# mct10/Speech-Vecalign

Hardware: AMD Instinct MI355X
Metric: aligned doc-pairs/sec (higher is better)
Workload: dtype bf16; 1 GPU; synthetic 4096x4096 d=1024 bf16 embeddings, 4 overlap layers/side, 10 alignment types, band 14, coarse-to-fine (max_size_full_dp=300), 1024 doc-pairs per GPU per step; pipeline=1, N=4096, M=4096, d=1024, overlaps=4, parallelism=dp1 (pairs sharded, no collective)

## Files before the change

### speech-vecalign_amd/csrc/svx_api.hip

```cpp
#include <stdarg.h>
#include <stdio.h>
#include <stdlib.h>
#include <string.h>

#include <chrono>
#include <functional>
#include <memory>
#include <type_traits>
#include <vector>

#include "svx_common.h"

static char g_err[512] = "";

int svx_fail(svx_ctx* ctx, int code, const char* fmt, ...) {
    char* dst = ctx ? ctx->err : g_err;
    va_list ap;
    va_start(ap, fmt);
    vsnprintf(dst, 512, fmt, ap);
    va_end(ap);
    return code;
}

static const char* kStageNames[] = {"pyr0",       "pyrN",     "pyr_aux",      "knob_scoresN", "knob",      "dense_costs",
// ... 796 lines not shown
static int next_event(svx_ctx* ctx, hipEvent_t* out) {
    svx_ctx_ext* cx = X(ctx);
    if (cx->ev_pool.size() < 256) {
        hipEvent_t e;
        SVX_HIP(ctx, hipEventCreateWithFlags(&e, hipEventDisableTiming));
        cx->ev_pool.push_back(e);
        *out = e;
        return SVX_OK;
    }
    *out = cx->ev_pool[cx->ev_next++ % cx->ev_pool.size()];
    return SVX_OK;
}

static void front_ops(svx_ctx* ctx, HalfState& H, std::vector<Op>& ops, int split) {
    svx_ctx_ext* cx = X(ctx);
    HalfState* h = &H;
    const BatchParams& bp = H.bp;
    const int np = H.n_pairs, d = bp.d, dtype = bp.dtype;
    const double waves = (double)((np + 1023) / 1024);
    const int parts = (split > 1 && np >= 16 * split) ? split : 1;
    struct Evs { hipEvent_t pass[SVX_MAX_LEVELS][8]; };
    auto evs = std::make_shared<Evs>();
    ops.push_back({0.0, -1, [=]() -> int {
        SVX_HIP(ctx, hipEventRecord(cx->side_fork, ctx->stream));
        SVX_HIP(ctx, hipStreamWaitEvent(cx->side, cx->side_fork, 0));
        SVX_HIP(ctx, hipStreamWaitEvent(cx->helper, cx->side_fork, 0));
        return SVX_OK;
    }});
    auto sort_op = [=]() -> int {
        hipStream_t main_stream = ctx->stream;
        static const bool inline_sort = getenv("SVX_SORT_INLINE") != nullptr;
        if (parts > 1 && !inline_sort) SVX_HIP(ctx, hipStreamWaitEvent(cx->side, evs->pass[0][parts - 1], 0));
        ctx->stream = inline_sort ? main_stream : cx->side;
        int rc;
        {
            StageScope sc(ctx, S_KNOB_SORT);
            rc = svxl_knob_scores(ctx, h->dpairs, np, h->maxL, h->max_kn, h->max_n0, dtype, d, 0);
        }
        ctx->stream = main_stream;
        if (rc) return rc;
        SVX_HIP(ctx, hipEventRecord(cx->side_join, inline_sort ? main_stream : cx->side));
        return SVX_OK;
    };
    if (parts == 1) ops.push_back({0.0, -1, sort_op});
    for (int l = 0; l <= H.maxL; l++) {
        for (int q = 0; q < parts; q++) {
            const int lo = (int)((long long)np * q / parts), hi = (int)((long long)np * (q + 1) / parts);
            const double aux_us = (l == 0 ? 700.0 * waves : 250.0) / parts;
            if (parts == 1) {
                ops.push_back({aux_us, S_PYR_AUX, [=]() { return svxl_pyramid_level(ctx, h->dpairs, np, l, dtype, d, h->max_nblk[l], h->max_ksum, 0); }});
                ops.push_back({H.b_pyr[l] / (l == 0 ? 4.9e6 : 5.3e6), l == 0 ? S_PYR0 : (l == 1 ? S_PYR1 : S_PYRN),
                               [=]() { return svxl_pyramid_level(ctx, h->dpairs, np, l, dtype, d, h->max_nblk[l], h->max_ksum, 1); }});
                continue;
            }
            ops.push_back({H.b_pyr[l] / (l == 0 ? 4.9e6 : 5.3e6) / parts, l == 0 ? S_PYR0 : (l == 1 ? S_PYR1 : S_PYRN), [=]() -> int {
                hipStream_t main_stream = ctx->stream;
                int rc;
                if (l == 0 && q == 0) {
                    StageScope sc(ctx, S_PYR_AUX);
                    if ((rc = svxl_pyramid_level(ctx, h->dpairs + lo, hi - lo, l, dtype, d, h->max_nblk[l], h->max_ksum, 0))) return rc;
                } else {
                    if (l > 0) SVX_HIP(ctx, hipStreamWaitEvent(cx->helper, evs->pass[l - 1][q], 0));
                    ctx->stream = cx->helper;
                    {
                        StageScope sc(ctx, S_PYR_AUX);
                        rc = svxl_pyramid_level(ctx, h->dpairs + lo, hi - lo, l, dtype, d, h->max_nblk[l], h->max_ksum, 0);
                    }
                    ctx->stream = main_stream;
                    if (rc) return rc;
                    hipEvent_t aux_done;
                    if ((rc = next_event(ctx, &aux_done))) return rc;
                    SVX_HIP(ctx, hipEventRecord(aux_done, cx->helper));
                    SVX_HIP(ctx, hipStreamWaitEvent(main_stream, aux_done, 0));
                }
                if ((rc = svxl_pyramid_level(ctx, h->dpairs + lo, hi - lo, l, dtype, d, h->max_nblk[l], h->max_ksum, 1))) return rc;
                if ((rc = next_event(ctx, &evs->pass[l][q]))) return rc;
                SVX_HIP(ctx, hipEventRecord(evs->pass[l][q], main_stream));
                return SVX_OK;
            }});
        }
        if (parts > 1 && l == 0) ops.push_back({0.0, -1, sort_op});
    }
    if (!bp.straight) {
        ops.push_back({H.dense_cells * 2.7e-5, S_DENSE_COSTS, [=]() -> int {
            int rc = svxl_dense_costs_batch(ctx, h->dpairs, np, h->max_ds0, h->max_ds1, dtype, d);
            if (rc) return rc;
            return svxl_knob_from_dots(ctx, h->dpairs, np, h->max_kn);
        }});
    }
    if (H.maxL >= 1) {
        ops.push_back({H.b_knobN / 16.5e6, S_KNOB_SCORES, [=]() -> int {
            SVX_HIP(ctx, hipStreamWaitEvent(ctx->stream, cx->side_join, 0));
            return svxl_knob_scores(ctx, h->dpairs, np, h->maxL, h->max_kn, h->max_n0, dtype, d, 1);
        }});
    }
    ops.push_back({H.b_knob0 / 8.5e6, S_KNOB_SCORES0, [=]() -> int {
        SVX_HIP(ctx, hipStreamWaitEvent(ctx->stream, cx->side_join, 0));
        return svxl_knob_scores(ctx, h->dpairs, np, h->maxL, h->max_kn, h->max_n0, dtype, d, 2);
    }});
}

struct Seg {
    std::vector<Op> lb;
    bool has_s = false;
    Op s;
};

static void chain_segs(svx_ctx* ctx, HalfState& H, std::vector<Seg>& segs) {
    HalfState* h = &H;
    const BatchParams bp = H.bp;
    const int np = H.n_pairs, d = bp.d, dtype = bp.dtype, W = bp.W, B = bp.B;
    const double waves = (double)((np + 1023) / 1024);
    Seg cur;
    cur.lb.push_back({(np * (H.maxL + 1) * 0.21 < 300.0 ? 300.0 : np * (H.maxL + 1) * 0.21), S_KNOB,
                      [=]() { return svxl_del_penalty_batch(ctx, h->dpairs, np, h->maxL + 1, bp.frac); }});
    if (!bp.straight)
        cur.lb.push_back({(H.max_ds0 + H.max_ds1) * 1.7 * waves, S_DENSE_DP, [=]() { return svxl_dense_stage_batch(ctx, h->dpairs, np, h->max_ds0); }});
    const int first_depth = H.maxL > 0 ? H.maxL - 1 : 0;
    for (int depth = first_depth; depth >= 0; depth--) {
        const SvxTypes ty = depth == 0 ? bp.tfinal : bp.t11;
        int lim2 = 0, tamax2 = 0;
        const bool v2 = !bp.tiles && svxl_band2_limits(ty, W, depth, dtype, d, &lim2, &tamax2);
        const int maxA = H.max_A[depth];
        const int src_rows = (H.maxL > 0 && !H.any_L0) ? maxA / 2 + 8 : maxA;
        cur.lb.push_back({maxA * 0.08 * waves + 60.0, depth == 0 ? S_PATH0 : S_PATH, [=]() {
            return svxl_search_path_batch(ctx, h->dpairs, np, depth, maxA, src_rows, v2 ? lim2 : SVX_BC_ROWS - SVX_BC_TB,
                                          bp.tiles ? 0 : (v2 ? tamax2 : SVX_BC_TAMAX));
        }});
        cur.has_s = true;
        if (bp.tiles) {
            cur.s = {1.0e4, S_TILES, [=]() {
                int* tk = reinterpret_cast<int*>(h->arena + h->o_tickets);
                float* planes = h->b_planes ? reinterpret_cast<float*>(h->arena + h->o_planes) : nullptr;
                return svxl_band_tiles_batch(ctx, h->dpairs, np, ty, W, dtype, h->max_tnd, tk, tk + (size_t)h->max_tnd * np + 1, planes);
            }};
        } else {
            cur.s = {H.b_bc[depth] / 4.0e6, depth == 0 ? S_BAND_COSTS0 : S_BAND_COSTSN, [=]() {
                return v2 ? svxl_band_costs2_batch(ctx, h->dpairs, np, depth, maxA, ty, W, dtype, d)
                          : svxl_band_costs_batch(ctx, h->dpairs, np, depth, maxA, ty, W, dtype, d);
            }};
        }
        segs.push_back(cur);
        cur = Seg();
        if (!bp.tiles)
            cur.lb.push_back({maxA * (0.21 + 0.054 * (ty.n > 1 ? ty.n : 0)) * waves, depth == 0 ? S_BAND_DP0 : S_BAND_DPN,
                              [=]() { return svxl_sparse_dp_batch(ctx, h->dpairs, np, depth, ty, B); }});
        cur.lb.push_back({maxA * 0.27 * waves, depth == 0 ? S_TRACEBACK0 : S_TRACEBACK, [=]() { return svxl_sparse_traceback_batch(ctx, h->dpairs, np, depth, B, maxA, bp.packable ? 1 : 0); }});
    }
    segs.push_back(cur);
}

static int ensure_streams(svx_ctx* ctx) {
    svx_ctx_ext* cx = X(ctx);
    if (!cx->side_ready) {
        int prio_lo = 0, prio_hi = 0;
        SVX_HIP(ctx, hipDeviceGetStreamPriorityRange(&prio_lo, &prio_hi));
        SVX_HIP(ctx, hipStreamCreateWithPriority(&cx->side, hipStreamNonBlocking, prio_lo));
        SVX_HIP(ctx, hipStreamCreateWithPriority(&cx->helper, hipStreamNonBlocking, prio_hi));
        SVX_HIP(ctx, hipEventCreateWithFlags(&cx->side_fork, hipEventDisableTiming));
        SVX_HIP(ctx, hipEventCreateWithFlags(&cx->side_join, hipEventDisableTiming));
        cx->side_ready = true;
    }
    if (!cx->chain_ready) {
        int prio_lo = 0, prio_hi = 0;
        SVX_HIP(ctx, hipDeviceGetStreamPriorityRange(&prio_lo, &prio_hi));
        SVX_HIP(ctx, hipStreamCreateWithPriority(&cx->chain, hipStreamNonBlocking, prio_hi));
        cx->chain_ready = true;
    }
    for (int h = 0; h < 2; h++) {
        if (!cx->half[h].front_done) SVX_HIP(ctx, hipEventCreateWithFlags(&cx->half[h].front_done, hipEventDisableTiming));
        if (!cx->half[h].chain_done) SVX_HIP(ctx, hipEventCreateWithFlags(&cx->half[h].chain_done, hipEventDisableTiming));
        if (!cx->half[h].upload_done) SVX_HIP(ctx, hipEventCreateWithFlags(&cx->half[h].upload_done, hipEventDisableTiming));
    }
    return SVX_OK;
}

static int run_interleaved(svx_ctx* ctx, HalfState* front, HalfState* chain, bool beside) {
    svx_ctx_ext* cx = X(ctx);
    hipStream_t A = ctx->stream, Bst = beside ? cx->chain : ctx->stream;
    std::vector<Op> fops;
    std::vector<Seg> segs;
    if (front) {
        if (front->chain_done_valid) SVX_HIP(ctx, hipStreamWaitEvent(A, front->chain_done, 0));
        {
            StageScope sc(ctx, S_SETUP);
            if (front->upload_valid) SVX_HIP(ctx, hipEventSynchronize(front->upload_done));
            memcpy(front->pinned, front->host.data(), (size_t)front->n_pairs * sizeof(SvxPairDev));
            SVX_HIP(ctx, hipMemcpyAsync(front->dpairs, front->pinned, (size_t)front->n_pairs * sizeof(SvxPairDev), hipMemcpyHostToDevice, A));
            SVX_HIP(ctx, hipEventRecord(front->upload_done, A));
            front->upload_valid = true;
            hipLaunchKernelGGL(k_init_batch, dim3(front->n_pairs), dim3(64), 0, A, front->dpairs);
            SVX_LAUNCH_CHECK(ctx, "k_init_batch");
            if (front->bp.around) {
                int rc = svxl_prior_ingest_batch(ctx, front->dpairs, front->n_pairs);
                if (rc) return rc;
            }
            if (front->bp.nsamp == 0) {
                for (int p = 0; p < front->n_pairs; p++)
                    for (int l = 0; l <= front->host[p].L; l++)
                        for (int s = 0; s < 2; s++)
                            SVX_HIP(ctx, hipMemsetAsync(front->host[p].lev[l].rbar[s], 0, (size_t)front->bp.d * sizeof(float), A));
            }
        }
        static const int split_env = [] { const char* e = getenv("SVX_PIPE_SPLIT"); const int v = e ? atoi(e) : 2; return v >= 1 && v <= 8 ? v : 2; }();
        front_ops(ctx, *front, fops, beside ? split_env : 1);
    }
    if (chain) chain_segs(ctx, *chain, segs);
    int rc;
    size_t fi = 0;
    if (chain && beside) SVX_HIP(ctx, hipStreamWaitEvent(Bst, chain->front_done, 0));
    for (size_t g = 0; g < segs.size(); g++) {
        double need = 0.0;
        for (const Op& op : segs[g].lb) {
            if ((rc = run_op(ctx, op, Bst))) return rc;
            need += op.us;
        }
        hipEvent_t lb_done = nullptr;
        if (beside) {
            if ((rc = next_event(ctx, &lb_done))) return rc;
            SVX_HIP(ctx, hipEventRecord(lb_done, Bst));
// ... 162 lines not shown
```

### speech-vecalign_amd/csrc/svx_band.hip

```cpp
#include <stdlib.h>
#include <string.h>

#include "svx_common.h"

namespace {

typedef __attribute__((ext_vector_type(8))) __bf16 bf16x8_t;
typedef __attribute__((ext_vector_type(8))) _Float16 f16x8_t;
typedef __attribute__((ext_vector_type(4))) float f32x4_t;
typedef __attribute__((address_space(1))) const void* gptr_t;
typedef __attribute__((address_space(3))) void* lptr_t;

constexpr int B2_THREADS = 256;
constexpr int B2_WAVES = 4;
constexpr int B2_TB = 16;
constexpr int B2_SLAB = 64;
constexpr int B2_MAXPASS = 8;
constexpr int B2_MAXSLOT = 20;
constexpr int B2_MAXTPP = 16;

__device__ const uint4 band_zero16[4] = {{0u, 0u, 0u, 0u}, {0u, 0u, 0u, 0u}, {0u, 0u, 0u, 0u}, {0u, 0u, 0u, 0u}};

struct BandPass {
    int t0, nt, nslot;
// ... 222 lines not shown
        auto step = [&](int k, const char* rd, char* wr) {
            if (k < NK) {
                const int younger = (NK - 1 - k) < (S - 2) ? (NK - 1 - k) : (S - 2);
                if (younger >= 2) wait_vm<2 * PW>();
                else if (younger == 1) wait_vm<PW>();
                else wait_vm<0>();
                __builtin_amdgcn_s_barrier();
                asm volatile("" ::: "memory");
                if (k + S - 1 < NK) issue(k + S - 1, wr);
                mma(rd);
            }
        };
        for (int k0 = 0; k0 < NK; k0 += S) {
            if (S == 2) {
                step(k0, st0, st1);
                step(k0 + 1, st1, st0);
            } else if (S == 3) {
                step(k0, st0, st2);
                step(k0 + 1, st1, st0);
                step(k0 + 2, st2, st1);
            } else {
                step(k0, st0, st3);
                step(k0 + 1, st1, st0);
                step(k0 + 2, st2, st1);
                step(k0 + 3, st3, st2);
            }
        }
#pragma unroll
        for (int i = 0; i < SPT; i++) {
            const int r = tid + i * B2_THREADS;
            if (r < NSLOT * ROWS) {
                snrm[r] = r_nrm[i];
                sinv[r] = r_inv[i];
            }
        }
        __syncthreads();
        const float inf = __builtin_inff();
#pragma unroll
        for (int s = 0; s < UPW; s++) {
            const int u = wave + B2_WAVES * s;
            if (u >= nunits) continue;
            const int tl = u / XT, xt = u % XT;
            const int p = ltx[ps.t0 + tl], q = lty[ps.t0 + tl];
            const int xs = (ps.type_slots[tl] & 255) * ROWS, ys = (ps.type_slots[tl] >> 8) * ROWS;
#pragma unroll
            for (int j = 0; j < XT; j++) {
                if (!((umask[s] >> j) & 1)) continue;
                const int yloc = 16 * j + lrow, yy = Y0 + yloc;
                const float ny = snrm[ys + yloc], iy = sinv[ys + yloc];
#pragma unroll
                for (int r = 0; r < 4; r++) {
                    const int xloc = 16 * xt + 4 * lkg + r, xx = X0 + xloc;
                    const int ai = xx + yy - a0;
                    if (ai < 0 || ai >= TAe) continue;
                    const int bi = yy - (spy[ai] - g.W) - b0;
                    if (bi < 0 || bi >= TBe) continue;
                    float c = inf;
                    if (xx >= 0 && xx < g.n && yy >= 0 && yy < g.m) {
                        const float sumx = acc[s][j][r] * sinv[xs + xloc] * iy;
                        c = cost_formula2(sumx, p, q, snrm[xs + xloc], ny);
                    }
                    Fs[(ai * ntp + tl) * TBe + bi] = c;
                }
            }
        }
        __syncthreads();
        if (TBe == B && ntp == g.T && ((g.T * B) & 3) == 0) {
            const int nv = TAe * ntp * TBe / 4;
            float4* dst = reinterpret_cast<float4*>(g.costs + (size_t)a0 * g.T * B);
            const float4* srcv = reinterpret_cast<const float4*>(Fs);
            for (int i = tid; i < nv; i += B2_THREADS) dst[i] = srcv[i];
        } else {
            const int nout = TAe * ntp * TBe;
            for (int idx = tid; idx < nout; idx += B2_THREADS) {
                const int ai = idx / (ntp * TBe);
                const int rem = idx - ai * (ntp * TBe);
                const int tl = rem / TBe, bi = rem - tl * TBe;
                g.costs[((size_t)(a0 + ai) * g.T + ps.t0 + tl) * B + (b0 + bi)] = Fs[idx];
            }
        }
    }
}

template <typename E, bool LV0, int ROWS, int NSLOT, int UPW, int S>
__global__ __launch_bounds__(B2_THREADS) void k_band_costs2(const SvxPairDev* __restrict__ pairs, int depth, SvxTypes ty, BandPlan plan,
                                                            int W, int nchunk_b, int per_pair) {
    using C = Band2<E, ROWS, NSLOT, UPW, S>;
    __shared__ __attribute__((aligned(1024))) char st0[C::STAGE];
    __shared__ __attribute__((aligned(1024))) char st1[C::STAGE];
    __shared__ __attribute__((aligned(1024))) char st2[S >= 3 ? C::STAGE : 16];
    __shared__ __attribute__((aligned(1024))) char st3[S >= 4 ? C::STAGE : 16];
    __shared__ __attribute__((aligned(16))) float Fs[C::FS_FLOATS];
    __shared__ int spx[C::TAMAX + 1], spy[C::TAMAX + 1];
    __shared__ float snrm[NSLOT * ROWS], sinv[NSLOT * ROWS];
    __shared__ int ltx[SVX_MAX_TYPES + 2], lty[SVX_MAX_TYPES + 2];
    __shared__ int tmask[C::XT];
    __shared__ int lslot[NSLOT];
    const unsigned wg = xcd_remap2(blockIdx.x, gridDim.x);
    const SvxPairDev& P = pairs[wg / per_pair];
    const int item = wg % per_pair;
    if (depth > P.L || (depth == P.L && P.L > 0)) return;
    const SvxLevel& Lv = P.lev[depth];
    Band2Args g;
    g.A = *Lv.path_len;
    const int chunk_a = item / nchunk_b;
    if (g.A <= 0 || chunk_a >= *Lv.nchunks) return;
    const int a0 = Lv.cstart[chunk_a], TAe = Lv.cstart[chunk_a + 1] - a0;
    if (TAe <= 0 || TAe > C::TAMAX) return;
    g.n = Lv.n[0];
    g.m = Lv.n[1];
    g.d = P.d;
    g.v0 = LV0 ? P.v[0] : (const void*)Lv.P[0];
    g.v1 = LV0 ? P.v[1] : (const void*)Lv.P[1];
    g.inv0 = LV0 ? Lv.inv[0] : nullptr;
    g.inv1 = LV0 ? Lv.inv[1] : nullptr;
    g.nrm0 = Lv.nrm[0];
    g.nrm1 = Lv.nrm[1];
    g.path = Lv.path;
    g.W = W;
    g.T = ty.n;
    g.costs = Lv.costs;
    g.boff = Lv.boff;
    g.status = P.status;
    band2_block<E, ROWS, NSLOT, UPW, S>(g, ty, plan, a0, TAe, item % nchunk_b, st0, st1, st2, st3, Fs, spx, spy, snrm, sinv, ltx, lty, tmask, lslot);
}

constexpr int B3_THREADS = 512, B3_ROWS = 32, B3_S = 8, B3_G = 2, B3_KX = 4, B3_KY = 4, B3_TMAX = 10;
constexpr int B3_STAGE = B3_KY * B3_ROWS * B2_SLAB;
constexpr int B3_FS = (2 * (B3_ROWS - B2_TB) + 1) * B2_TB * B3_TMAX;

struct BandPlan3 {
    int kx, ky;
    int wt_n[B3_KX];
    int wt_type[B3_KX][B3_KY];
    int wt_yl[B3_KX][B3_KY];
};

template <typename E, int NK, bool AASM, int G>
__device__ void band3_block(const Band2Args& g, const BandPlan3& plan, int a0, int TAe, int chunk_b, char* ring, float* Fs, int* spx,
                            int* spy, float* snrm, float* sinv) {
    using St = typename E::storage;
    static_assert(sizeof(St) == 2, "16-bit rows");
    constexpr int ROWS = B3_ROWS, S = B3_S;
    const int tid = threadIdx.x, lane = tid & 63;
    const int wave = __builtin_amdgcn_readfirstlane(tid >> 6);
    const int xl = wave >> 1, xt = wave & 1;
    const int B = 2 * g.W, b0 = chunk_b * B2_TB;
    const int TBe = (B - b0) < B2_TB ? (B - b0) : B2_TB;
    constexpr int rowbytes = NK * B2_SLAB;
    const int kx = plan.kx, ky = plan.ky;

    if (tid < TAe) {
        const int2 p = reinterpret_cast<const int2*>(g.path)[a0 + tid];
        spx[tid] = p.x;
        spy[tid] = p.y;
    }
    __syncthreads();
    if (tid < TAe) {
        bool ok = (spx[tid] + spy[tid] == a0 + tid);
        if (tid > 0) ok = ok && spx[tid] >= spx[tid - 1] && spy[tid] >= spy[tid - 1];
        if (!ok && g.status) *g.status = SVX_ERR_PATH;
        if (chunk_b == 0) g.boff[a0 + tid] = spy[tid] - g.W;
    }
    const int xlo = spx[0], ylo = spy[0];
    const int X0 = xlo + g.W - (b0 + TBe - 1);
    const int Y0 = ylo - g.W + b0;
    int NXn = spx[TAe - 1] - xlo + TBe, NYn = spy[TAe - 1] - ylo + TBe;
    NXn = NXn < 1 ? 1 : (NXn > ROWS ? ROWS : NXn);
    NYn = NYn < 1 ? 1 : (NYn > ROWS ? ROWS : NYn);

    float r_nrm = 0.f, r_inv = 1.f;
    if (tid < 2 * B3_KX * ROWS) {
        const int side = tid >= B3_KX * ROWS, rr = tid - side * B3_KX * ROWS;
        const int layer = rr / ROWS, loc = rr % ROWS;
        const int gi = (side ? Y0 : X0) + loc, nn = side ? g.m : g.n;
// ... 187 lines not shown
    float* Fs = reinterpret_cast<float*>(ring);
    __shared__ int spx[2 * B3_ROWS], spy[2 * B3_ROWS];
    __shared__ float snrm[2 * B3_KX * B3_ROWS], sinv[2 * B3_KX * B3_ROWS];
    const unsigned wg = xcd_remap2(blockIdx.x, gridDim.x);
    const SvxPairDev& P = pairs[wg / per_pair];
    const int item = wg % per_pair;
    const SvxLevel& Lv = P.lev[0];
    Band2Args g;
    g.A = *Lv.path_len;
    const int chunk_a = item / nchunk_b;
    if (g.A <= 0 || chunk_a >= *Lv.nchunks) return;
    const int a0 = Lv.cstart[chunk_a], TAe = Lv.cstart[chunk_a + 1] - a0;
    if (TAe <= 0 || TAe > 2 * (B3_ROWS - 1) + 1) return;
    g.n = Lv.n[0];
    g.m = Lv.n[1];
    g.d = P.d;
    g.v0 = P.v[0];
    g.v1 = P.v[1];
    g.inv0 = Lv.inv[0];
    g.inv1 = Lv.inv[1];
    g.nrm0 = Lv.nrm[0];
    g.nrm1 = Lv.nrm[1];
    g.path = Lv.path;
    g.W = W;
    g.T = T;
    g.costs = Lv.costs;
    g.boff = Lv.boff;
    g.status = P.status;
    band3_block<E, NK, AASM, G>(g, plan, a0, TAe, item % nchunk_b, ring, Fs, spx, spy, snrm, sinv);
}

bool make_plan3(const SvxTypes& ty, BandPlan3* plan) {
    memset(plan, 0, sizeof(*plan));
    if (ty.n < 1 || ty.n > B3_TMAX) return false;
    for (int t = 0; t < ty.n; t++) {
        const int lx = ty.x[t] - 1, ly = ty.y[t] - 1;
        if (lx >= B3_KX || ly >= B3_KY) return false;
        if (plan->wt_n[lx] >= B3_KY) return false;
        plan->wt_type[lx][plan->wt_n[lx]] = t;
        plan->wt_yl[lx][plan->wt_n[lx]] = ly;
        plan->wt_n[lx]++;
        if (lx + 1 > plan->kx) plan->kx = lx + 1;
        if (ly + 1 > plan->ky) plan->ky = ly + 1;
    }
    return true;
}

int band_version() {
    const char* env = getenv("SVX_BAND_V");
    return env ? atoi(env) : 3;
}

bool make_plan(const SvxTypes& ty, int tpp, int nslot_max, BandPlan* plan) {
    plan->npass = 0;
    int t = 0;
    while (t < ty.n) {
        if (plan->npass >= B2_MAXPASS) return false;
        BandPass& ps = plan->pass[plan->npass];
        memset(&ps, 0, sizeof(ps));
        ps.t0 = t;
        int xs[SVX_MAX_TYPES + 2], ys[SVX_MAX_TYPES + 2];
        memset(xs, 0, sizeof(xs));
        memset(ys, 0, sizeof(ys));
        while (t < ty.n && ps.nt < tpp) {
            const int lx = ty.x[t] - 1, ly = ty.y[t] - 1;
            const int need = (xs[lx] ? 0 : 1) + (ys[ly] ? 0 : 1);
            if (ps.nslot + need > nslot_max) break;
            if (!xs[lx]) { ps.slot_info[ps.nslot] = lx; xs[lx] = ++ps.nslot; }
            if (!ys[ly]) { ps.slot_info[ps.nslot] = (1 << 8) | ly; ys[ly] = ++ps.nslot; }
            ps.type_slots[ps.nt] = (xs[lx] - 1) | ((ys[ly] - 1) << 8);
            ps.nt++;
            t++;
        }
        if (ps.nt == 0) return false;
        plan->npass++;
    }
    return true;
}

struct Variant {
    int rows, nslot, upw, s;
};

bool choose_variant(const SvxTypes& ty, int depth, Variant* v, BandPlan* plan) {
    if (ty.n <= 0) return false;
    int kx = 0, ky = 0;
    for (int t = 0; t < ty.n; t++) {
        if (ty.x[t] > kx) kx = ty.x[t];
        if (ty.y[t] > ky) ky = ty.y[t];
    }
    (void)depth;
    const Variant opts[4] = {{64, 2, 1, 4}, {32, 8, 5, 3}, {32, 12, 8, 3}, {32, 20, 8, 2}};
    for (int i = 0; i < 4; i++) {
        const int tpp = B2_WAVES * opts[i].upw / (opts[i].rows / 16);
        const bool last = i == 3;
        if (!last && (kx + ky > opts[i].nslot || ty.n > tpp)) continue;
        if (!make_plan(ty, tpp, opts[i].nslot, plan)) continue;
        *v = opts[i];
        return true;
    }
    return false;
}

}

static bool use_v3(const SvxTypes& types, int depth, int dtype, int d, BandPlan3* plan3) {
    const int nk3 = d / 32;
    return depth == 0 && dtype != SVX_F32 && band_version() >= 3 && d % 32 == 0 && (nk3 == 32 || nk3 == 16 || nk3 == 8) &&
           make_plan3(types, plan3);
}

bool svxl_band2_limits(const SvxTypes& types, int W, int depth, int dtype, int d, int* lim, int* tamax) {
    const char* env = getenv("SVX_BAND_V1");
    if ((env && atoi(env) != 0) || band_version() <= 1) return false;
    const char* deep = getenv("SVX_BAND_DEEP_V1");
    if (depth > 0 && deep && atoi(deep) != 0) return false;
    Variant v;
    BandPlan plan;
    BandPlan3 plan3;
    if (use_v3(types, depth, dtype, d, &plan3)) v.rows = B3_ROWS;
    else if (!choose_variant(types, depth, &v, &plan)) return false;
    const int B = 2 * W, tbe = B < B2_TB ? B : B2_TB;
    *lim = v.rows - tbe;
    *tamax = 2 * (v.rows - tbe) + 1;
    return true;
}

int svxl_band_costs2_batch(svx_ctx* ctx, const SvxPairDev* pairs, int n_pairs, int depth, int max_A, const SvxTypes& types, int W,
                           int dtype, int d) {
    if (n_pairs <= 0 || max_A <= 0) return SVX_OK;
    BandPlan3 plan3;
    const int nk3 = d / 32;
    if (use_v3(types, depth, dtype, d, &plan3)) {
        const int B3 = 2 * W, tbe3 = B3 < B2_TB ? B3 : B2_TB, lim3 = B3_ROWS - tbe3;
        const int nca3 = (max_A + lim3) / (lim3 + 1), ncb3 = (B3 + B2_TB - 1) / B2_TB;
        dim3 grid3((unsigned)(nca3 * ncb3) * (unsigned)n_pairs);
        const char* aenv = getenv("SVX_BAND_ASMLOAD");
        const bool aasm = aenv ? atoi(aenv) != 0 : true;
#define CALL3(E, NKT)                                                                                                             \
    do {                                                                                                                          \
        if (aasm) hipLaunchKernelGGL((k_band_costs3<E, NKT, true, B3_G>), grid3, dim3(B3_THREADS), 0, ctx->stream, pairs, plan3, types.n, W, ncb3, nca3 * ncb3); \
        else hipLaunchKernelGGL((k_band_costs3<E, NKT, false, B3_G>), grid3, dim3(B3_THREADS), 0, ctx->stream, pairs, plan3, types.n, W, ncb3, nca3 * ncb3); \
    } while (0)
#define CALL3_E(E)                      \
    do {                                \
        if (nk3 == 32) CALL3(E, 32);    \
        else if (nk3 == 16) CALL3(E, 16); \
        else CALL3(E, 8);               \
    } while (0)
        if (dtype == SVX_F16) CALL3_E(ElemF16);
        else CALL3_E(ElemBF16);
#undef CALL3_E
#undef CALL3
        SVX_LAUNCH_CHECK(ctx, "k_band_costs3");
        return SVX_OK;
    }
    Variant v;
    BandPlan plan;
    if (!choose_variant(types, depth, &v, &plan)) return svx_fail(ctx, SVX_ERR_ARG, "band costs: no kernel shape for %d alignment types", types.n);
    const int B = 2 * W, tbe = B < B2_TB ? B : B2_TB;
    const int lim = v.rows - tbe;
    const int nca = (max_A + lim) / (lim + 1), ncb = (B + B2_TB - 1) / B2_TB;
    const int per_pair = nca * ncb;
    dim3 grid((unsigned)per_pair * (unsigned)n_pairs);
    hipStream_t st = ctx->stream;
#define CALL2(E, LV0, ROWS, NSLOT, UPW, S) \
    hipLaunchKernelGGL((k_band_costs2<E, LV0, ROWS, NSLOT, UPW, S>), grid, dim3(B2_THREADS), 0, st, pairs, depth, types, plan, W, ncb, per_pair)
#define CALL2_V(E, LV0)                                      \
    do {                                                     \
        if (v.nslot == 2) CALL2(E, LV0, 64, 2, 1, 4);        \
        else if (v.nslot == 8) CALL2(E, LV0, 32, 8, 5, 3);   \
        else if (v.nslot == 12) CALL2(E, LV0, 32, 12, 8, 3); \
        else CALL2(E, LV0, 32, 20, 8, 2);                    \
    } while (0)
    if (depth > 0) CALL2_V(ElemF32, false);
    else if (dtype == SVX_F32) CALL2_V(ElemF32, true);
    else if (dtype == SVX_F16) CALL2_V(ElemF16, true);
    else CALL2_V(ElemBF16, true);
#undef CALL2_V
#undef CALL2
    SVX_LAUNCH_CHECK(ctx, "k_band_costs2");
    return SVX_OK;
}
```

### speech-vecalign_amd/csrc/svx_costs.hip

```cpp
#include <stdlib.h>

#include "svx_common.h"

namespace {

typedef __attribute__((ext_vector_type(8))) __bf16 bf16x8_t;
typedef __attribute__((ext_vector_type(8))) _Float16 f16x8_t;
typedef __attribute__((ext_vector_type(4))) float f32x4_t;

constexpr int RS = 144;

template <typename E>
struct Mma;
template <>
struct Mma<ElemBF16> {
    static constexpr int KS = 64, NK = 2, KSTEP_BYTES = 64;
    using frag = uint4;
    __device__ static __forceinline__ int lane_off(int lane) { return (lane & 15) * RS + 16 * (lane >> 4); }
    __device__ static __forceinline__ frag load(const char* p) { return *reinterpret_cast<const uint4*>(p); }
    __device__ static __forceinline__ void mma(f32x4_t& acc, const frag& a, const frag& b) {
        acc = __builtin_amdgcn_mfma_f32_16x16x32_bf16(__builtin_bit_cast(bf16x8_t, a), __builtin_bit_cast(bf16x8_t, b), acc, 0, 0, 0);
    }
};
template <>
// ... 57 lines not shown
    const int tid = threadIdx.x, lane = tid & 63, wave = tid >> 6;
    const char** rowptr = reinterpret_cast<const char**>(smem);
    char* slab = smem + 2 * DT * sizeof(char*);
    const int x0 = bx * DT, y0 = by * DT;
    if (tid < 2 * DT) {
        const int side = tid >= DT, loc = tid - side * DT;
        const int gi = (side ? y0 : x0) + loc;
        const int nn = side ? g.s1 : g.s0;
        const char* base = reinterpret_cast<const char*>(side ? g.v1 : g.v0);
        rowptr[tid] = (gi < nn) ? base + (size_t)gi * g.d * sizeof(S) : nullptr;
    }
    f32x4_t acc[2][2];
#pragma unroll
    for (int i = 0; i < 2; i++)
#pragma unroll
        for (int j = 0; j < 2; j++) acc[i][j] = (f32x4_t){0.f, 0.f, 0.f, 0.f};
    const int xt = wave >> 1, yt = wave & 1;
    for (int k0 = 0; k0 < g.d; k0 += Mma<E>::KS) {
        __syncthreads();
        stage_slab<E>(slab, rowptr, 2 * DT, k0, g.d, tid, blockDim.x);
        __syncthreads();
        const char* ap = slab + xt * 32 * RS + Mma<E>::lane_off(lane);
        const char* bp = slab + (DT + yt * 32) * RS + Mma<E>::lane_off(lane);
#pragma unroll
        for (int ks = 0; ks < Mma<E>::NK; ks++) {
            const typename Mma<E>::frag a0 = Mma<E>::load(ap + ks * Mma<E>::KSTEP_BYTES);
            const typename Mma<E>::frag a1 = Mma<E>::load(ap + 16 * RS + ks * Mma<E>::KSTEP_BYTES);
            const typename Mma<E>::frag b0 = Mma<E>::load(bp + ks * Mma<E>::KSTEP_BYTES);
            const typename Mma<E>::frag b1 = Mma<E>::load(bp + 16 * RS + ks * Mma<E>::KSTEP_BYTES);
            Mma<E>::mma(acc[0][0], a0, b0);
            Mma<E>::mma(acc[0][1], a0, b1);
            Mma<E>::mma(acc[1][0], a1, b0);
            Mma<E>::mma(acc[1][1], a1, b1);
        }
    }
#pragma unroll
    for (int i = 0; i < 2; i++)
#pragma unroll
        for (int j = 0; j < 2; j++) {
            const int y = y0 + yt * 32 + j * 16 + (lane & 15);
#pragma unroll
            for (int r = 0; r < 4; r++) {
                const int x = x0 + xt * 32 + i * 16 + (lane >> 4) * 4 + r;
                if (x < g.s0 && y < g.s1) {
                    float sumx = acc[i][j][r];
                    if (g.inv0) sumx = sumx * g.inv0[x] * g.inv1[y];
                    float c = cost_formula(sumx, 1, 1, g.n0[x], g.n1[y]);
                    c = (c * (float)g.mul0) * (float)g.mul1;
                    g.costs[(size_t)x * g.s1 + y] = c;
                    if (g.dots) g.dots[(size_t)x * g.s1 + y] = sumx;
                }
            }
        }
}

template <typename E>
__global__ __launch_bounds__(256) void k_dense_costs(DenseArgs g) {
    extern __shared__ __attribute__((aligned(16))) char smem[];
    dense_block<E>(g, blockIdx.x, blockIdx.y, smem);
}

template <typename E, bool LV0>
__global__ __launch_bounds__(256) void k_dense_costs_batch(const SvxPairDev* __restrict__ pairs) {
    extern __shared__ __attribute__((aligned(16))) char smem[];
    const SvxPairDev& P = pairs[blockIdx.z];
    if ((P.L == 0) != LV0) return;
    const SvxLevel& Lv = P.lev[P.L];
    DenseArgs g;
    g.s0 = Lv.n[0];
    g.s1 = Lv.n[1];
    if ((int)blockIdx.x * DT >= g.s0 || (int)blockIdx.y * DT >= g.s1) return;
    g.d = P.d;
    g.v0 = LV0 ? P.v[0] : (const void*)Lv.P[0];
    g.v1 = LV0 ? P.v[1] : (const void*)Lv.P[1];
    g.inv0 = LV0 ? Lv.inv[0] : nullptr;
    g.inv1 = LV0 ? Lv.inv[1] : nullptr;
    g.n0 = Lv.nrm[0];
    g.n1 = Lv.nrm[1];
    g.mul0 = 1;
    g.mul1 = 1;
    g.costs = P.dcost;
    g.dots = LV0 ? nullptr : P.ddot;
    dense_block<E>(g, blockIdx.x, blockIdx.y, smem);
}

template <typename E, int NCH>
__device__ __forceinline__ float row_dot(const typename E::storage* a, const typename E::storage* b, int d, int lane) {
    float s = 0.f;
#pragma unroll
    for (int c = 0; c < NCH; c++) {
        const int col = (c * SVX_WAVE + lane) * E::VEC;
        if (col < d) {
            float x[E::VEC], y[E::VEC];
            load_piece<E>(a + col, x);
            load_piece<E>(b + col, y);
#pragma unroll
            for (int i = 0; i < E::VEC; i++) s += x[i] * y[i];
        }
    }
    return wave_sum(s);
}

struct ScoreArgs {
    const void* v1;
    const void* v2;
    const float* inv1;
    const float* inv2;
    const float* n1;
    const float* n2;
    const int* xx;
    const int* yy;
    int64_t n;
    int rows1, rows2, d;
    float* out;
};

template <typename E, int NCH>
__device__ void score_block(const ScoreArgs& g, int64_t first, int64_t stride) {
    using S = typename E::storage;
    const int lane = threadIdx.x & 63;
    for (int64_t i = first; i < g.n; i += stride) {
        int xi = g.xx[i], yi = g.yy[i];
        xi = xi < 0 ? 0 : (xi >= g.rows1 ? g.rows1 - 1 : xi);
        yi = yi < 0 ? 0 : (yi >= g.rows2 ? g.rows2 - 1 : yi);
        float dot = row_dot<E, NCH>(reinterpret_cast<const S*>(g.v1) + (size_t)xi * g.d,
                                    reinterpret_cast<const S*>(g.v2) + (size_t)yi * g.d, g.d, lane);
        if (lane == 0) {
            if (g.inv1) dot = dot * g.inv1[xi] * g.inv2[yi];
            const float den = g.n1[xi] + g.n2[yi];
            g.out[i] = (float)((2.0 * (1.0 - (double)dot)) / (double)den);
        }
    }
}

template <typename E, int NCH>
__global__ __launch_bounds__(256) void k_score_path(ScoreArgs g) {
    score_block<E, NCH>(g, (int64_t)blockIdx.x * 4 + (threadIdx.x >> 6), (int64_t)gridDim.x * 4);
}

__device__ __forceinline__ unsigned xcd_remap(unsigned id, unsigned n);

__global__ __launch_bounds__(256) void k_knob_sort(const SvxPairDev* __restrict__ pairs) {
    extern __shared__ __attribute__((aligned(16))) char smem[];
    __shared__ int part[256];
    const SvxPairDev& P = pairs[blockIdx.y];
    const int level = blockIdx.x;
    if (level > P.L) return;
    if (P.L >= 1 && level == P.L) return;
    const SvxLevel& Lv = P.lev[level];
    const int n = Lv.n[0], kn = Lv.kn, tid = threadIdx.x;
    int* cnt = reinterpret_cast<int*>(smem);
    for (int i = tid; i < n; i += 256) cnt[i] = 0;
    __syncthreads();
    for (int i = tid; i < kn; i += 256) {
        int x = Lv.kx[i];
        x = x < 0 ? 0 : (x >= n ? n - 1 : x);
        atomicAdd(&cnt[x], 1);
    }
    __syncthreads();
    const int per = (n + 255) / 256;
    const int lo = tid * per, hi = (lo + per) < n ? (lo + per) : n;
    int sum = 0;
    for (int i = lo; i < hi; i++) sum += cnt[i];
    part[tid] = sum;
    __syncthreads();
    if (tid == 0) {
// ... 438 lines not shown
        }
        const int nout = TAe * ntp * TBe;
        for (int idx = tid; idx < nout; idx += BC_THREADS) {
            const int ai = idx / (ntp * TBe);
            const int rem = idx - ai * (ntp * TBe);
            const int tl = rem / TBe, bi = rem - tl * TBe;
            const int t = pass * TPP + tl;
            const size_t o = g.atb ? ((size_t)(a0 + ai) * ty.n + t) * B + (b0 + bi) : ((size_t)t * g.A + (a0 + ai)) * B + (b0 + bi);
            g.costs[o] = Fs[((size_t)ai * ntp + tl) * TB + bi];
        }
    }
}

template <typename E, int NPT, int SW>
__global__ __launch_bounds__(BC_THREADS) void k_band_costs(BandArgs g, SvxTypes ty, int kx, int ky, int nchunk_b) {
    extern __shared__ __attribute__((aligned(16))) char smem[];
    const int a0 = (blockIdx.x / nchunk_b) * TA;
    band_block<E, NPT, SW>(g, ty, kx, ky, a0, (g.A - a0) < TA ? (g.A - a0) : TA, blockIdx.x % nchunk_b, smem);
}

__device__ __forceinline__ unsigned xcd_remap(unsigned id, unsigned n) {
    const unsigned q = n / 8, r = n % 8, xcd = id % 8, k = id / 8;
    return (xcd < r ? xcd * (q + 1) : r * (q + 1) + (xcd - r) * q) + k;
}

template <typename E, bool LV0, int NPT, int SW>
__global__ __launch_bounds__(BC_THREADS) void k_band_costs_batch(const SvxPairDev* __restrict__ pairs, int depth, SvxTypes ty,
                                                                 int kx, int ky, int W, int nchunk_b, int per_pair) {
    extern __shared__ __attribute__((aligned(16))) char smem[];
    const unsigned wg = xcd_remap(blockIdx.x, gridDim.x);
    const SvxPairDev& P = pairs[wg / per_pair];
    const int item = wg % per_pair;
    if (depth > P.L || (depth == P.L && P.L > 0)) return;
    const SvxLevel& Lv = P.lev[depth];
    BandArgs g;
    g.A = *Lv.path_len;
    const int chunk_a = item / nchunk_b;
    if (g.A <= 0 || chunk_a >= *Lv.nchunks) return;
    const int a0 = Lv.cstart[chunk_a], TAe = Lv.cstart[chunk_a + 1] - a0;
    g.n = Lv.n[0];
    g.m = Lv.n[1];
    g.d = P.d;
    g.v0 = LV0 ? P.v[0] : (const void*)Lv.P[0];
    g.v1 = LV0 ? P.v[1] : (const void*)Lv.P[1];
    g.inv0 = LV0 ? Lv.inv[0] : nullptr;
    g.inv1 = LV0 ? Lv.inv[1] : nullptr;
    g.nrm0 = Lv.nrm[0];
    g.nrm1 = Lv.nrm[1];
    g.path = Lv.path;
    g.W = W;
    g.costs = Lv.costs;
    g.boff = Lv.boff;
    g.status = P.status;
    g.atb = 1;
    band_block<E, NPT, SW>(g, ty, kx, ky, a0, TAe, item % nchunk_b, smem);
}

inline int nch_f32(int d) {
    int c = (d + 255) / 256;
    return c <= 1 ? 1 : c <= 2 ? 2 : c <= 4 ? 4 : 8;
}
inline int nch_16(int d) {
    int c = (d + 511) / 512;
    return c <= 1 ? 1 : c <= 2 ? 2 : 4;
}

constexpr size_t DENSE_SMEM = 2 * DT * sizeof(char*) + 2 * DT * RS;

}

int svxl_dense_costs(svx_ctx* ctx, const float* v0, int s0, const float* v1, int s1, int d, const float* n0,
                     const float* n1, int mul0, int mul1, float* costs) {
    if (s0 <= 0 || s1 <= 0) return SVX_OK;
    DenseArgs g{v0, v1, s0, s1, d, nullptr, nullptr, n0, n1, mul0, mul1, costs, nullptr};
    hipLaunchKernelGGL(k_dense_costs<ElemF32>, dim3((s0 + DT - 1) / DT, (s1 + DT - 1) / DT), dim3(256), DENSE_SMEM, ctx->stream, g);
    SVX_LAUNCH_CHECK(ctx, "k_dense_costs");
    return SVX_OK;
}

int svxl_dense_costs_batch(svx_ctx* ctx, const SvxPairDev* pairs, int n_pairs, int max_s0, int max_s1, int dtype, int d) {
    (void)d;
    if (n_pairs <= 0 || max_s0 <= 0 || max_s1 <= 0) return SVX_OK;
    dim3 grid((max_s0 + DT - 1) / DT, (max_s1 + DT - 1) / DT, n_pairs);
    hipLaunchKernelGGL((k_dense_costs_batch<ElemF32, false>), grid, dim3(256), DENSE_SMEM, ctx->stream, pairs);
    if (dtype == SVX_F32)
        hipLaunchKernelGGL((k_dense_costs_batch<ElemF32, true>), grid, dim3(256), DENSE_SMEM, ctx->stream, pairs);
    else if (dtype == SVX_F16)
        hipLaunchKernelGGL((k_dense_costs_batch<ElemF16, true>), grid, dim3(256), DENSE_SMEM, ctx->stream, pairs);
    else
        hipLaunchKernelGGL((k_dense_costs_batch<ElemBF16, true>), grid, dim3(256), DENSE_SMEM, ctx->stream, pairs);
    SVX_LAUNCH_CHECK(ctx, "k_dense_costs_batch");
    return SVX_OK;
}

int svxl_score_path(svx_ctx* ctx, const int* xx, const int* yy, int64_t n, const float* n1, const float* n2,
                    const float* v1, int rows1, const float* v2, int rows2, int d, float* out) {
    if (n <= 0) return SVX_OK;
    ScoreArgs g{v1, v2, nullptr, nullptr, n1, n2, xx, yy, n, rows1, rows2, d, out};
    int64_t nb = (n + 3) / 4;
    if (nb > 16384) nb = 16384;
#define M(N) hipLaunchKernelGGL((k_score_path<ElemF32, N>), dim3((unsigned)nb), dim3(256), 0, ctx->stream, g)
    switch (nch_f32(d)) {
        case 1: M(1); break;
        case 2: M(2); break;
        case 4: M(4); break;
        default: M(8); break;
    }
#undef M
    SVX_LAUNCH_CHECK(ctx, "k_score_path");
    return SVX_OK;
}

int svxl_knob_from_dots(svx_ctx* ctx, const SvxPairDev* pairs, int n_pairs, int max_kn) {
    if (n_pairs <= 0 || max_kn <= 0) return SVX_OK;
    int nb = (max_kn + 255) / 256;
    if (nb > 16) nb = 16;
    hipLaunchKernelGGL(k_knob_from_dots, dim3(nb, n_pairs), dim3(256), 0, ctx->stream, pairs);
    SVX_LAUNCH_CHECK(ctx, "k_knob_from_dots");
    return SVX_OK;
}

int svxl_knob_scores(svx_ctx* ctx, const SvxPairDev* pairs, int n_pairs, int max_L, int max_kn, int max_n0, int dtype, int d,
                     int part) {
    if (n_pairs <= 0 || max_kn <= 0) return SVX_OK;
    hipStream_t st = ctx->stream;
    const bool unsorted = (size_t)(max_n0 + 1) * sizeof(int) > 150 * 1024;
    if (unsorted) {
        if (part == 0) return SVX_OK;
        const int nbu = (max_kn + 3) / 4 < 2048 ? (max_kn + 3) / 4 : 2048;
#define U32(N, LV0, GY) hipLaunchKernelGGL((k_knob_scores_unsorted<ElemF32, N, LV0>), dim3(nbu, GY, n_pairs), dim3(256), 0, st, pairs)
#define U16(E, N) hipLaunchKernelGGL((k_knob_scores_unsorted<E, N, true>), dim3(nbu, 1, n_pairs), dim3(256), 0, st, pairs)
        if (part == 1) {
            if (max_L >= 1) {
                switch (nch_f32(d)) {
                    case 1: U32(1, false, max_L); break;
                    case 2: U32(2, false, max_L); break;
                    case 4: U32(4, false, max_L); break;
                    default: U32(8, false, max_L); break;
                }
            }
        } else if (dtype == SVX_F32) {
            switch (nch_f32(d)) {
                case 1: U32(1, true, 1); break;
                case 2: U32(2, true, 1); break;
                case 4: U32(4, true, 1); break;
                default: U32(8, true, 1); break;
            }
        } else if (dtype == SVX_F16) {
            switch (nch_16(d)) {
                case 1: U16(ElemF16, 1); break;
                case 2: U16(ElemF16, 2); break;
                default: U16(ElemF16, 4); break;
            }
        } else {
            switch (nch_16(d)) {
                case 1: U16(ElemBF16, 1); break;
                case 2: U16(ElemBF16, 2); break;
                default: U16(ElemBF16, 4); break;
            }
        }
#undef U32
#undef U16
        SVX_LAUNCH_CHECK(ctx, "k_knob_scores_unsorted");
        return SVX_OK;
    }
    if (part == 0) {
        const size_t smem = (size_t)(max_n0 + 1) * sizeof(int);
// ... 175 lines not shown
```

Before: 9636 doc-pairs/s.

## Add MFMA-pipelined dense cost kernel for coarse levels and reuse stage LDS for output

Adds a new dense-cost kernel for non-zero pyramid levels that streams 128x128 tiles through a four-stage global_load_lds pipeline with swizzled LDS and fp32 MFMA 16x16x4 accumulation, replacing the older dense_block path (the old one stays behind an env var). The deep band-cost kernel for nslot==2 now aliases its output image onto the first stage buffer, cutting LDS use so more workgroups can be resident. Scheduler cost estimates are retuned to match. The cost is more hand-written inline asm with fixed vmcnt assumptions and a four-stage LDS budget.

```diff
diff --git a/speech-vecalign_amd/csrc/svx_api.hip b/speech-vecalign_amd/csrc/svx_api.hip
--- a/speech-vecalign_amd/csrc/svx_api.hip
+++ b/speech-vecalign_amd/csrc/svx_api.hip
@@ -902,7 +902,7 @@
         if (parts > 1 && l == 0) ops.push_back({0.0, -1, sort_op});
     }
     if (!bp.straight) {
-        ops.push_back({H.dense_cells * 2.7e-5, S_DENSE_COSTS, [=]() -> int {
+        ops.push_back({H.dense_cells * 2.5e-5, S_DENSE_COSTS, [=]() -> int {
             int rc = svxl_dense_costs_batch(ctx, h->dpairs, np, h->max_ds0, h->max_ds1, dtype, d);
             if (rc) return rc;
             return svxl_knob_from_dots(ctx, h->dpairs, np, h->max_kn);
@@ -955,7 +955,7 @@
                 return svxl_band_tiles_batch(ctx, h->dpairs, np, ty, W, dtype, h->max_tnd, tk, tk + (size_t)h->max_tnd * np + 1, planes);
             }};
         } else {
-            cur.s = {H.b_bc[depth] / 4.0e6, depth == 0 ? S_BAND_COSTS0 : S_BAND_COSTSN, [=]() {
+            cur.s = {H.b_bc[depth] / (depth == 0 ? 4.0e6 : 3.5e6), depth == 0 ? S_BAND_COSTS0 : S_BAND_COSTSN, [=]() {
                 return v2 ? svxl_band_costs2_batch(ctx, h->dpairs, np, depth, maxA, ty, W, dtype, d)
                           : svxl_band_costs_batch(ctx, h->dpairs, np, depth, maxA, ty, W, dtype, d);
             }};
diff --git a/speech-vecalign_amd/csrc/svx_band.hip b/speech-vecalign_amd/csrc/svx_band.hip
--- a/speech-vecalign_amd/csrc/svx_band.hip
+++ b/speech-vecalign_amd/csrc/svx_band.hip
@@ -328,15 +328,17 @@
     }
 }
 
-template <typename E, bool LV0, int ROWS, int NSLOT, int UPW, int S>
+template <typename E, bool LV0, int ROWS, int NSLOT, int UPW, int S, bool FSR = false>
 __global__ __launch_bounds__(B2_THREADS) void k_band_costs2(const SvxPairDev* __restrict__ pairs, int depth, SvxTypes ty, BandPlan plan,
                                                             int W, int nchunk_b, int per_pair) {
     using C = Band2<E, ROWS, NSLOT, UPW, S>;
+    static_assert(!FSR || C::FS_FLOATS * sizeof(float) <= (size_t)C::STAGE, "output image inside a stage");
     __shared__ __attribute__((aligned(1024))) char st0[C::STAGE];
     __shared__ __attribute__((aligned(1024))) char st1[C::STAGE];
     __shared__ __attribute__((aligned(1024))) char st2[S >= 3 ? C::STAGE : 16];
     __shared__ __attribute__((aligned(1024))) char st3[S >= 4 ? C::STAGE : 16];
-    __shared__ __attribute__((aligned(16))) float Fs[C::FS_FLOATS];
+    __shared__ __attribute__((aligned(16))) float Fsown[FSR ? 4 : C::FS_FLOATS];
+    float* Fs = FSR ? reinterpret_cast<float*>(st0) : Fsown;
     __shared__ int spx[C::TAMAX + 1], spy[C::TAMAX + 1];
     __shared__ float snrm[NSLOT * ROWS], sinv[NSLOT * ROWS];
     __shared__ int ltx[SVX_MAX_TYPES + 2], lty[SVX_MAX_TYPES + 2];
@@ -690,6 +692,11 @@
     int rows, nslot, upw, s;
 };
 
+bool deep_own_image() {
+    const char* e = getenv("SVX_BAND_DEEP_OWNFS");
+    return e && atoi(e) != 0;
+}
+
 bool choose_variant(const SvxTypes& ty, int depth, Variant* v, BandPlan* plan) {
     if (ty.n <= 0) return false;
     int kx = 0, ky = 0;
@@ -781,7 +788,9 @@
         else if (v.nslot == 12) CALL2(E, LV0, 32, 12, 8, 3); \
         else CALL2(E, LV0, 32, 20, 8, 2);                    \
     } while (0)
-    if (depth > 0) CALL2_V(ElemF32, false);
+    if (depth > 0 && v.nslot == 2 && !deep_own_image()) {
+        hipLaunchKernelGGL((k_band_costs2<ElemF32, false, 64, 2, 1, 4, true>), grid, dim3(B2_THREADS), 0, st, pairs, depth, types, plan, W, ncb, per_pair);
+    } else if (depth > 0) CALL2_V(ElemF32, false);
     else if (dtype == SVX_F32) CALL2_V(ElemF32, true);
     else if (dtype == SVX_F16) CALL2_V(ElemF16, true);
     else CALL2_V(ElemBF16, true);
diff --git a/speech-vecalign_amd/csrc/svx_costs.hip b/speech-vecalign_amd/csrc/svx_costs.hip
--- a/speech-vecalign_amd/csrc/svx_costs.hip
+++ b/speech-vecalign_amd/csrc/svx_costs.hip
@@ -163,6 +163,154 @@
     g.costs = P.dcost;
     g.dots = LV0 ? nullptr : P.ddot;
     dense_block<E>(g, blockIdx.x, blockIdx.y, smem);
+}
+
+typedef __attribute__((address_space(1))) const void* d2_gptr_t;
+typedef __attribute__((address_space(3))) void* d2_lptr_t;
+constexpr int D2_T = 128, D2_S = 4, D2_SLAB = 64, D2_THREADS = 256;
+constexpr int D2_STAGE = 2 * D2_T * D2_SLAB;
+constexpr int D2_PW = 2 * D2_T / 16 / 4;
+static_assert(D2_PW * (D2_S - 2) <= 63, "vmcnt is a 6-bit counter");
+
+__device__ const uint4 dense_zero16[4] = {{0u, 0u, 0u, 0u}, {0u, 0u, 0u, 0u}, {0u, 0u, 0u, 0u}, {0u, 0u, 0u, 0u}};
+
+template <int N>
+__device__ __forceinline__ void d2_wait_vm() {
+    asm volatile("s_waitcnt vmcnt(%0)" ::"n"(N) : "memory");
+}
+__device__ __forceinline__ int d2_swz(int row_in_tile) { return (0x1320 >> (4 * ((row_in_tile >> 2) & 3))) & 3; }
+
+__device__ __forceinline__ unsigned xcd_remap(unsigned id, unsigned n);
+
+__global__ __launch_bounds__(D2_THREADS) void k_dense_costs_batch2(const SvxPairDev* __restrict__ pairs, int nbx, int per_pair) {
+    __shared__ __attribute__((aligned(1024))) char st0[D2_STAGE];
+    __shared__ __attribute__((aligned(1024))) char st1[D2_STAGE];
+    __shared__ __attribute__((aligned(1024))) char st2[D2_STAGE];
+    __shared__ __attribute__((aligned(1024))) char st3[D2_STAGE];
+    static_assert(D2_S == 4, "four stage objects");
+    const unsigned wg = xcd_remap(blockIdx.x, gridDim.x);
+    const SvxPairDev& P = pairs[wg / per_pair];
+    const int item = wg % per_pair;
+    if (P.L == 0) return;
+    const SvxLevel& Lv = P.lev[P.L];
+    const int s0 = Lv.n[0], s1 = Lv.n[1];
+    const int x0 = (item % nbx) * D2_T, y0 = (item / nbx) * D2_T;
+    if (x0 >= s0 || y0 >= s1) return;
+    const int tid = threadIdx.x, lane = tid & 63;
+    const int wave = __builtin_amdgcn_readfirstlane(tid >> 6);
+    const int rowbytes = P.d * (int)sizeof(float);
+    const int NK = (rowbytes + D2_SLAB - 1) / D2_SLAB;
+
+    const int piece_byte = ((lane & 3) ^ d2_swz(lane >> 2)) * 16;
+    const char* src[D2_PW];
+    unsigned live = 0;
+#pragma unroll
+    for (int i = 0; i < D2_PW; i++) {
+        const int r = 16 * (wave + 4 * i) + (lane >> 2);
+        const int side = r >= D2_T, gi = (side ? y0 - D2_T : x0) + r;
+        src[i] = reinterpret_cast<const char*>(dense_zero16);
+        if (gi < (side ? s1 : s0)) {
+            src[i] = reinterpret_cast<const char*>(side ? Lv.P[1] : Lv.P[0]) + (size_t)gi * rowbytes + piece_byte;
+            live |= 1u << i;
+        }
+    }
+    auto issue = [&](int k, char* stage) {
+#pragma unroll
+        for (int i = 0; i < D2_PW; i++) {
+            const char* s = src[i] + (size_t)k * D2_SLAB;
+            if (!((live >> i) & 1u) || k * D2_SLAB + piece_byte >= rowbytes) s = reinterpret_cast<const char*>(dense_zero16);
+            __builtin_amdgcn_global_load_lds((d2_gptr_t)s, (d2_lptr_t)(stage + (wave + 4 * i) * 1024), 16, 0, 0);
+        }
+    };
+    f32x4_t acc[4][4];
+#pragma unroll
+    for (int i = 0; i < 4; i++)
+#pragma unroll
+        for (int j = 0; j < 4; j++) acc[i][j] = (f32x4_t){0.f, 0.f, 0.f, 0.f};
+    const int xt = wave >> 1, yt = wave & 1;
+    const int lrow = lane & 15, lkg = lane >> 4;
+    const unsigned abase = xt * 64 * D2_SLAB + lrow * D2_SLAB + 4 * lkg;
+    const unsigned bbase = (D2_T + yt * 64) * D2_SLAB + lrow * D2_SLAB + 4 * lkg;
+    const int sw = d2_swz(lrow);
+    auto mma = [&](const char* stage) {
+        const unsigned sb = (unsigned)(size_t)(d2_lptr_t)const_cast<char*>(stage);
+#pragma unroll
+        for (int h = 0; h < 2; h++) {
+            const unsigned p0 = 16 * ((2 * h) ^ sw), p1 = 16 * ((2 * h + 1) ^ sw);
+            float a[2][4], b[2][4];
+            asm volatile(
+                "ds_read_b32 %0, %16\n\tds_read_b32 %1, %16 offset:1024\n\tds_read_b32 %2, %16 offset:2048\n\tds_read_b32 %3, %16 offset:3072\n\t"
+                "ds_read_b32 %4, %17\n\tds_read_b32 %5, %17 offset:1024\n\tds_read_b32 %6, %17 offset:2048\n\tds_read_b32 %7, %17 offset:3072\n\t"
+                "ds_read_b32 %8, %18\n\tds_read_b32 %9, %18 offset:1024\n\tds_read_b32 %10, %18 offset:2048\n\tds_read_b32 %11, %18 offset:3072\n\t"
+                "ds_read_b32 %12, %19\n\tds_read_b32 %13, %19 offset:1024\n\tds_read_b32 %14, %19 offset:2048\n\tds_read_b32 %15, %19 offset:3072\n\t"
+                "s_waitcnt lgkmcnt(0)"
+                : "=&v"(a[0][0]), "=&v"(a[0][1]), "=&v"(a[0][2]), "=&v"(a[0][3]), "=&v"(b[0][0]), "=&v"(b[0][1]), "=&v"(b[0][2]), "=&v"(b[0][3]),
+                  "=&v"(a[1][0]), "=&v"(a[1][1]), "=&v"(a[1][2]), "=&v"(a[1][3]), "=&v"(b[1][0]), "=&v"(b[1][1]), "=&v"(b[1][2]), "=&v"(b[1][3])
+                : "v"(sb + abase + p0), "v"(sb + bbase + p0), "v"(sb + abase + p1), "v"(sb + bbase + p1)
+                : "memory");
+#pragma unroll
+            for (int ks = 0; ks < 2; ks++)
+#pragma unroll
+                for (int i = 0; i < 4; i++)
+#pragma unroll
+                    for (int j = 0; j < 4; j++) acc[i][j] = __builtin_amdgcn_mfma_f32_16x16x4f32(a[ks][i], b[ks][j], acc[i][j], 0, 0, 0);
+        }
+    };
+    if (0 < NK) issue(0, st0);
+    if (1 < NK) issue(1, st1);
+    if (2 < NK) issue(2, st2);
+    auto step = [&](int k, const char* rd, char* wr) {
+        if (k < NK) {
+            const int younger = (NK - 1 - k) < (D2_S - 2) ? (NK - 1 - k) : (D2_S - 2);
+            if (younger >= 2) d2_wait_vm<2 * D2_PW>();
+            else if (younger == 1) d2_wait_vm<D2_PW>();
+            else d2_wait_vm<0>();
+            __builtin_amdgcn_s_barrier();
+            asm volatile("" ::: "memory");
+            if (k + D2_S - 1 < NK) issue(k + D2_S - 1, wr);
+            mma(rd);
+        }
+    };
+    for (int k0 = 0; k0 < NK; k0 += D2_S) {
+        step(k0, st0, st3);
+        step(k0 + 1, st1, st0);
+        step(k0 + 2, st2, st1);
+        step(k0 + 3, st3, st2);
+    }
+    float* __restrict__ costs = P.dcost;
+    float* __restrict__ dots = P.ddot;
+    const float* __restrict__ n0 = Lv.nrm[0];
+    const float* __restrict__ n1 = Lv.nrm[1];
+    float nx[4][4], ny[4];
+#pragma unroll
+    for (int i = 0; i < 4; i++)
+#pragma unroll
+        for (int r = 0; r < 4; r++) {
+            const int x = x0 + xt * 64 + i * 16 + lkg * 4 + r;
+            nx[i][r] = n0[x < s0 ? x : s0 - 1];
+        }
+#pragma unroll
+    for (int j = 0; j < 4; j++) {
+        const int y = y0 + yt * 64 + j * 16 + lrow;
+        ny[j] = n1[y < s1 ? y : s1 - 1];
+    }
+#pragma unroll
+    for (int j = 0; j < 4; j++) {
+        const int y = y0 + yt * 64 + j * 16 + lrow;
+        if (y >= s1) continue;
+#pragma unroll
+        for (int i = 0; i < 4; i++) {
+#pragma unroll
+            for (int r = 0; r < 4; r++) {
+                const int x = x0 + xt * 64 + i * 16 + lkg * 4 + r;
+                if (x < s0) {
+                    const float sumx = acc[i][j][r];
+                    costs[(size_t)x * s1 + y] = cost_formula(sumx, 1, 1, nx[i][r], ny[j]);
+                    dots[(size_t)x * s1 + y] = sumx;
+                }
+            }
+        }
+    }
 }
 
 template <typename E, int NCH>
@@ -767,7 +915,14 @@
     (void)d;
     if (n_pairs <= 0 || max_s0 <= 0 || max_s1 <= 0) return SVX_OK;
     dim3 grid((max_s0 + DT - 1) / DT, (max_s1 + DT - 1) / DT, n_pairs);
-    hipLaunchKernelGGL((k_dense_costs_batch<ElemF32, false>), grid, dim3(256), DENSE_SMEM, ctx->stream, pairs);
+    const char* v1env = getenv("SVX_DENSE_V1");
+    if (v1env && atoi(v1env) != 0) {
+        hipLaunchKernelGGL((k_dense_costs_batch<ElemF32, false>), grid, dim3(256), DENSE_SMEM, ctx->stream, pairs);
+    } else {
+        const int nbx = (max_s0 + D2_T - 1) / D2_T, nby = (max_s1 + D2_T - 1) / D2_T;
+        hipLaunchKernelGGL(k_dense_costs_batch2, dim3((unsigned)(nbx * nby) * (unsigned)n_pairs), dim3(D2_THREADS), 0, ctx->stream, pairs, nbx,
+                           nbx * nby);
+    }
     if (dtype == SVX_F32)
         hipLaunchKernelGGL((k_dense_costs_batch<ElemF32, true>), grid, dim3(256), DENSE_SMEM, ctx->stream, pairs);
     else if (dtype == SVX_F16)
```

New measurement: 9706 doc-pairs/s, median of 6. Within noise of the previous version (+0.7%).
